# rusty1s/pytorch_sparse

Measured on AMD Instinct MI355X. Metric: SpMM GEdges/s, higher is better.
Workload: dtype f32; 1 GPU; north-star: CSR SpMM 2M x 2M R-MAT ~20 nnz/row, F=128 fp32; reduce=sum, rows_per_gpu=2097152, cols=2097152, edges_per_gpu=40294089, features=128, parallelism=row-sharded x1

## Files before the change

### include/tsamd.h

```cpp
#ifndef TSAMD_H_
#define TSAMD_H_

#include <stddef.h>
#include <stdint.h>

#ifdef __cplusplus
extern "C" {
#endif

typedef enum {
  TSAMD_OK = 0,
  TSAMD_ERR_INVALID = 1,
  TSAMD_ERR_UNSUPPORTED = 2,
  TSAMD_ERR_HIP = 3,
  TSAMD_ERR_WORKSPACE = 4
} tsamd_status;

typedef enum {
  TSAMD_F32 = 0,
  TSAMD_F64 = 1,
  TSAMD_F16 = 2,
  TSAMD_BF16 = 3,
  TSAMD_I32 = 4,
  TSAMD_I64 = 5,
// ... 7 lines not shown
int64_t tsamd_hip_version(void);
int tsamd_build_flags(void);
int tsamd_last_hip_error(void);
const char *tsamd_status_string(int status);

size_t tsamd_spmm_workspace_bytes(int dtype, int reduce, int64_t B, int64_t M,
                                  int64_t N, int64_t K, int64_t E);

int tsamd_spmm_hot_rows_layout(int dtype, int reduce, int64_t B, int64_t M, int64_t N, int64_t K, int64_t E,
                               const void *mat, const void *out, void *workspace, int64_t *layout);

int tsamd_spmm_hot_blocks_layout(int dtype, int reduce, int64_t B, int64_t M, int64_t N, int64_t K, int64_t E,
                                 const void *mat, const void *out, void *workspace, int64_t *layout);
int tsamd_spmm_hot_block_min(void);

int tsamd_spmm_route(int dtype, int reduce, int64_t B, int64_t M, int64_t N, int64_t K, int64_t E, const void *mat,
                     const void *out, const void *arg_out, int arg32, void *workspace, int64_t route[24]);

int tsamd_spmm(int dtype, int reduce, const int64_t *rowptr, const int64_t *col,
               const void *value, const void *mat, void *out, int64_t *arg_out,
               int64_t B, int64_t M, int64_t N, int64_t K, int64_t E,
               void *workspace, size_t workspace_bytes, void *stream);
int tsamd_spmm_reference_order(int set);

int tsamd_spmm_permuted(int dtype, int reduce, const int64_t *rowptr, const int64_t *col,
                        const void *value, const int64_t *perm, const void *mat, void *out,
                        int64_t *arg_out, int64_t B, int64_t M, int64_t N, int64_t K, int64_t E,
                        void *workspace, size_t workspace_bytes, void *stream);

size_t tsamd_spmm_partial_workspace_bytes(int dtype, int reduce, int64_t B, int64_t M, int64_t N, int64_t K,
                                          int64_t E);
int tsamd_spmm_partial(int dtype, int reduce, const int64_t *rowptr, const int64_t *col, const void *value,
                       const void *mat, void *out, int64_t *arg_out, int64_t B, int64_t M, int64_t N, int64_t K,
                       int64_t E, const int64_t *arg_map, int64_t arg_none, int accumulate,
                       const int64_t *deg_rowptr, void *workspace, size_t workspace_bytes, void *stream);

size_t tsamd_spmm_operand_cache_bytes(int dtype, int reduce, int64_t B, int64_t M, int64_t N, int64_t K,
                                      int64_t E);
size_t tsamd_spmm_cached_workspace_bytes(int dtype, int reduce, int64_t B, int64_t M, int64_t N, int64_t K,
                                         int64_t E);
int tsamd_spmm_cached(int dtype, int reduce, const int64_t *rowptr, const int64_t *col, const void *value,
                      const void *mat, void *out, int64_t *arg_out, int64_t B, int64_t M, int64_t N,
                      int64_t K, int64_t E, void *workspace, size_t workspace_bytes, void *cache,
                      size_t cache_bytes, int cache_valid, void *stream);

int tsamd_spmm_profiled(int dtype, int reduce, const int64_t *rowptr,
// ... 349 lines not shown
```

### pytorch_sparse_amd/_native.py

```python
import ctypes
import os

import torch

_HERE = os.path.dirname(os.path.abspath(__file__))
LIB_PATH = os.environ.get('TSAMD_LIB') or os.path.join(_HERE, 'lib', 'libtsamd.so')

SYMBOLS = [
    'tsamd_hip_version', 'tsamd_build_flags', 'tsamd_last_hip_error', 'tsamd_status_string',
    'tsamd_spmm_workspace_bytes', 'tsamd_spmm_hot_rows_layout', 'tsamd_spmm_hot_blocks_layout', 'tsamd_spmm_hot_block_min', 'tsamd_spmm_route', 'tsamd_spmm', 'tsamd_spmm_reference_order', 'tsamd_spmm_permuted', 'tsamd_spmm_profiled',
    'tsamd_spmm_partial_workspace_bytes', 'tsamd_spmm_partial',
    'tsamd_spmm_operand_cache_bytes', 'tsamd_spmm_cached_workspace_bytes', 'tsamd_spmm_cached',
    'tsamd_spmm_minmax_arg32', 'tsamd_spmm_minmax_bw_csc_arg32',
    'tsamd_spmm_minmax_records_in_forward', 'tsamd_spmm_minmax_records_bytes', 'tsamd_spmm_minmax_records_workspace_bytes', 'tsamd_spmm_minmax_records',
    'tsamd_spmm_minmax_winrec', 'tsamd_spmm_minmax_bw_csc_records_workspace_bytes', 'tsamd_spmm_minmax_bw_csc_records',
    'tsamd_gather_rows', 'tsamd_relabel_ids', 'tsamd_spmm_relabelled_workspace_bytes', 'tsamd_spmm_relabelled',
    'tsamd_spmm_coo_small_supported', 'tsamd_spmm_coo_small',
    'tsamd_spmm_value_bw',
    'tsamd_spmm_minmax_bw_workspace_bytes', 'tsamd_spmm_minmax_bw',
    'tsamd_spmm_minmax_bw_csc_workspace_bytes', 'tsamd_spmm_minmax_bw_csc', 'tsamd_spmm_minmax_bw_route',
    'tsamd_ind2ptr', 'tsamd_ptr2ind',
    'tsamd_coo_order', 'tsamd_coo_check', 'tsamd_sort_rank_mode', 'tsamd_sort_route', 'tsamd_sort_coalesce_workspace_bytes', 'tsamd_sort_coalesce', 'tsamd_sort_coalesce_reduce', 'tsamd_sort_coo_workspace_bytes', 'tsamd_sort_coo', 'tsamd_sort_coo_auto', 'tsamd_sort_coo_probed', 'tsamd_sort_coo_values',
    'tsamd_coalesce_workspace_bytes', 'tsamd_coalesce_index', 'tsamd_segment_reduce',
    'tsamd_segment_reduce_balanced_workspace_bytes', 'tsamd_segment_reduce_balanced',
    'tsamd_segment_softmax_route', 'tsamd_segment_softmax_workspace_bytes', 'tsamd_segment_softmax', 'tsamd_segment_softmax_bw',
    'tsamd_sddmm_heads_route', 'tsamd_sddmm_heads', 'tsamd_spmm_heads_route', 'tsamd_spmm_heads_workspace_bytes', 'tsamd_spmm_heads',
    'tsamd_exclusive_scan_workspace_bytes', 'tsamd_exclusive_scan_i64',
    'tsamd_spspmm_route', 'tsamd_spspmm_plan', 'tsamd_spspmm_workspace_bytes', 'tsamd_spspmm_symbolic', 'tsamd_spspmm_numeric',
    'tsamd_spspmm_bw_route', 'tsamd_spspmm_bw_plan_workspace_bytes', 'tsamd_spspmm_bw_workspace_bytes', 'tsamd_spspmm_bw_plan', 'tsamd_spspmm_value_bw',
    'tsamd_index_route', 'tsamd_select_workspace_bytes', 'tsamd_select_plan', 'tsamd_select_fill',
    'tsamd_filter_workspace_bytes', 'tsamd_filter_plan', 'tsamd_filter_apply',
    'tsamd_filter_tiles_workspace_bytes', 'tsamd_filter_count', 'tsamd_filter_write',
    'tsamd_scatter_rows',
# ... 142 lines not shown
    check(st, 'tsamd_spmm')
    return out, arg


SPMM_ROUTE_FIELDS = ('family', 'vec', 'slots', 'lpr', 'lgG', 'ktiles', 'P', 'items', 'snap', 'relabel', 'copy', 'fixup',
                     'table_off', 'tail_row_off', 'head_row_off', 'relabel_flag_off', 'records', 'grid_y',
                     'workspace_bytes')
SPMM_FAMILIES = ('none', 'short', 'cooperative', 'hot_rows', 'hot_blocks', 'arg32_short', 'arg32_cooperative',
                 'reference_order')


def spmm_route(dtype, reduce, B, M, N, K, E, mat=0, out=0, arg_out=0, arg32=False, workspace=0):
    def addr(p):
        return ctypes.c_void_p(int(p.data_ptr() if hasattr(p, 'data_ptr') else p))
    words = (ctypes.c_int64 * 24)()
    st = lib().tsamd_spmm_route(dtype_code(dtype), REDUCES[reduce], _i64(B), _i64(M), _i64(N), _i64(K), _i64(E), addr(mat),
                                addr(out), addr(arg_out), ctypes.c_int(1 if arg32 else 0), addr(workspace), words)
    check(st, 'tsamd_spmm_route')
    r = dict(zip(SPMM_ROUTE_FIELDS, (int(x) for x in words)))
    r['family'] = SPMM_FAMILIES[r['family']]
    return r


def spmm_partial(rowptr, col, value, mat, reduce, out, arg_out=None, arg_map=None, arg_none=0, accumulate=True,
                 deg_rowptr=None):
    require_gpu(rowptr, col, value, mat, out, arg_out, arg_map, deg_rowptr)
    red = REDUCES[reduce]
    dt = dtype_code(mat.dtype)
    if value is not None and value.dtype != mat.dtype:
        raise TsamdError('expected scalar type %s but found %s' % (mat.dtype, value.dtype))
    if not (mat.is_contiguous() and out.is_contiguous() and (arg_out is None or arg_out.is_contiguous())):
        raise TsamdError('tsamd_spmm_partial works in place: mat / out / arg_out must be contiguous')
    if out.dtype != mat.dtype or (red >= 2 and (arg_out is None or arg_out.dtype != torch.int64)):
        raise TsamdError('Input mismatch: out / arg_out')
    M, E = rowptr.numel() - 1, col.numel()
    N, K = mat.size(-2), mat.size(-1)
    B = mat.numel() // max(N * K, 1) if N * K > 0 else 1
    if out.numel() != B * M * K or (arg_out is not None and arg_out.numel() != out.numel()):
        raise TsamdError('Input mismatch: out must be [B, M, K]')
    L = lib()
    nb = L.tsamd_spmm_partial_workspace_bytes(dt, red, _i64(B), _i64(M), _i64(N), _i64(K), _i64(E))
    ws = workspace(nb, mat.device)
    with torch.cuda.device(mat.device):
        st = L.tsamd_spmm_partial(dt, red, _ptr(rowptr), _ptr(col), _ptr(value), _ptr(mat), _ptr(out), _ptr(arg_out),
                                  _i64(B), _i64(M), _i64(N), _i64(K), _i64(E), _ptr(arg_map), _i64(arg_none),
                                  ctypes.c_int(1 if accumulate else 0), _ptr(deg_rowptr), _ptr(ws),
# ... 264 lines not shown
```

### pytorch_sparse_amd/csrc/ops_spmm.cpp

```cpp
#include "ops_common.h"

namespace tsamd_ops {
namespace {

bool stream_is_capturing(void *stream) {
  hipStreamCaptureStatus cs = hipStreamCaptureStatusNone;
  return hipStreamIsCapturing(reinterpret_cast<hipStream_t>(stream), &cs) != hipSuccess ||
         cs != hipStreamCaptureStatusNone;
}

struct TensorIdentity {
  c10::weak_intrusive_ptr<c10::StorageImpl> storage{c10::weak_intrusive_ptr<c10::StorageImpl>(
      c10::make_intrusive<c10::StorageImpl>(c10::StorageImpl::use_byte_size_t(), 0, c10::DataPtr(), nullptr, false))};
  const void *ptr = nullptr;
  uint32_t version = 0;

  static uint32_t version_of(const Tensor &t) { return t.unsafeGetTensorImpl()->version_counter().current_version(); }
  bool matches(const Tensor &t) const {
    if (ptr != t.data_ptr() || version != version_of(t)) return false;
    auto alive = storage.lock();
    return alive && alive.get() == t.storage().unsafeGetStorageImpl();
  }
  void rearm(const Tensor &t) {
    storage = c10::weak_intrusive_ptr<c10::StorageImpl>(
// ... 696 lines not shown

Tensor spmm_coo_small(Tensor index, Tensor value, int64_t M, int64_t N, Tensor mat) {
  if (!(index.device().is_cuda() && value.device().is_cuda() && mat.device().is_cuda()) || mat.dim() != 2 ||
      index.dim() != 2 || index.size(0) != 2 || index.scalar_type() != at::kLong || value.dim() != 1 ||
      value.size(0) != index.size(1) || value.scalar_type() != mat.scalar_type() || mat.size(0) != N ||
      !spmm_coo_small_supported(value, index.size(1), M, mat.size(1)))
    return torch::empty({0}, mat.options().requires_grad(false));
  c10::hip::HIPGuard guard(mat.get_device());
  index = index.contiguous();
  value = value.contiguous();
  mat = mat.contiguous();
  const int64_t E = index.size(1), K = mat.size(1);
  Tensor out = torch::empty({M, K}, mat.options().requires_grad(false));
  check_status(tsamd_spmm_coo_small(dtype_code(mat), index.data_ptr<int64_t>(), index.data_ptr<int64_t>() + E,
                                    value.data_ptr(), mat.data_ptr(), out.data_ptr(), E, M, N, K, current_stream(mat)),
               "tsamd_spmm_coo_small");
  return out;
}

int64_t cuda_version() { return tsamd_hip_version(); }

int64_t reference_order(int64_t set) { return (int64_t)tsamd_spmm_reference_order((int)set); }

bool deterministic_mode() { return at::globalContext().deterministicAlgorithms(); }


}
}

using namespace tsamd_ops;

static auto registry_spmm = torch::RegisterOperators()
                           .op("torch_sparse::spmm_sum", &spmm_sum)
                           .op("torch_sparse::spmm_mean", &spmm_mean)
                           .op("torch_sparse::spmm_min", &spmm_min)
                           .op("torch_sparse::spmm_max", &spmm_max)
                           .op("torch_sparse::ind2ptr", &ind2ptr)
                           .op("torch_sparse::ptr2ind", &ptr2ind)
                           .op("torch_sparse::cuda_version", &cuda_version)
                           .op("tsamd::spmm_coo_small", &spmm_coo_small)
                           .op("tsamd::spmm_coo_small_supported", &spmm_coo_small_supported)
                           .op("tsamd::spmm_minmax", &spmm_minmax)
                           .op("tsamd::deterministic", &deterministic_mode)
                           .op("tsamd::reference_order", &reference_order)
                           .op("tsamd::spmm_sum_owned", &spmm_sum_owned)
                           .op("tsamd::spmm_mean_owned", &spmm_mean_owned)
                           .op("tsamd::operand_cache", &operand_cache_ctl)
                           .op("tsamd::pattern_cache", &pattern_cache_ctl)
                           .op("tsamd::pattern_cache_stats", &pattern_cache_stats)
                           .op("tsamd::relabel_ids", &relabel_ids)
                           .op("tsamd::gather_rows", &gather_rows)
                           .op("tsamd::spmm_relabelled", &spmm_relabelled);
```

### pytorch_sparse_amd/csrc/spmm.hip

```cpp
#define TSAMD_SPMM_PARTIAL_BUILD 0
#include "spmm_kernels.h"

using namespace tsamd;

static int spmm_run(const SpmmCall &c) {
  return spmm_entry(c, [&](int vec, const Workspace &ws) -> int {
    if (c.reduce == TSAMD_MIN) return spmm_launch_min(vec, c, ws);
    if (c.reduce == TSAMD_MAX) return spmm_launch_max(vec, c, ws);
    return TSAMD_DISPATCH_DTYPE_ALL(c.dtype, [&]() -> int { return dispatch_spmm<scalar_t, RED_ADD>(vec, c, ws); });
  });
}

extern "C" size_t tsamd_spmm_workspace_bytes(int dtype, int reduce, int64_t B, int64_t M,
                                             int64_t N, int64_t K, int64_t E) {
  if (dtype_size(dtype) == 0 || B < 0 || M < 0 || N < 0 || K < 0 || E < 0) return 0;
  return carve(nullptr, dtype, reduce, B, M, N, K, E, nullptr);
}

extern "C" int tsamd_spmm(int dtype, int reduce, const int64_t *rowptr, const int64_t *col,
                          const void *value, const void *mat, void *out, int64_t *arg_out,
                          int64_t B, int64_t M, int64_t N, int64_t K, int64_t E, void *workspace,
                          size_t workspace_bytes_given, void *stream_) {
  return spmm_run(SpmmCall{dtype, reduce, rowptr, col, value, mat, out, arg_out, B, M, N, K, E, workspace,
                           workspace_bytes_given, reinterpret_cast<hipStream_t>(stream_)});
// ... 12 lines not shown
  if ((K * es) % packet != 0 || (uintptr_t)mat % packet != 0 || (uintptr_t)out % packet != 0) return 0;
  void *side = nullptr;
  int32_t side_row = 0;
  if (!hot_rows_place(ws, mat, blocks ? N + 64 : N, (uint64_t)K * es, &side, &side_row)) return 0;
  const char *base = reinterpret_cast<const char *>(workspace);
  layout[0] = reinterpret_cast<const char *>(ws.hot_flag) - base;
  layout[1] = reinterpret_cast<const char *>(blocks ? ws.blk_word : ws.hot_word) - base;
  layout[2] = reinterpret_cast<const char *>(side) - base;
  layout[3] = side_row;
  return 1;
}

extern "C" int tsamd_spmm_hot_rows_layout(int dtype, int reduce, int64_t B, int64_t M, int64_t N, int64_t K, int64_t E,
                                          const void *mat, const void *out, void *workspace, int64_t *layout) {
  return hot_layout(false, dtype, reduce, B, M, N, K, E, mat, out, workspace, layout);
}

extern "C" int tsamd_spmm_hot_blocks_layout(int dtype, int reduce, int64_t B, int64_t M, int64_t N, int64_t K, int64_t E,
                                            const void *mat, const void *out, void *workspace, int64_t *layout) {
  return hot_layout(true, dtype, reduce, B, M, N, K, E, mat, out, workspace, layout);
}

extern "C" int tsamd_spmm_hot_block_min(void) { return kHotBlockMin; }

static bool spmm_emits_records(int dtype, int64_t B, int64_t M, int64_t K, int64_t E, const void *mat, const void *out);

int tsamd::spmm_route_words(int dtype, int reduce, int64_t B, int64_t M, int64_t N, int64_t K, int64_t E, const void *mat,
                            const void *out, const void *arg_out, int arg32, void *workspace, bool masked,
                            int64_t route[24]) {
  if (!route || B < 0 || M < 0 || N < 0 || K < 0 || E < 0) return TSAMD_ERR_INVALID;
  for (int i = 0; i < 24; ++i) route[i] = 0;
  if (reduce < TSAMD_SUM || reduce > TSAMD_MAX) return TSAMD_ERR_UNSUPPORTED;
  if (dtype_size(dtype) == 0) return TSAMD_ERR_UNSUPPORTED;
  if (N >= (int64_t)1 << 32 || K >= (int64_t)1 << 31 || B >= 65536) return TSAMD_ERR_UNSUPPORTED;
  if (B * ceil_div(K, 64) >= 65536) return TSAMD_ERR_UNSUPPORTED;
  const bool minmax = reduce == TSAMD_MIN || reduce == TSAMD_MAX;
  const bool floating = dtype == TSAMD_F32 || dtype == TSAMD_F64 || dtype == TSAMD_F16 || dtype == TSAMD_BF16;
  if (arg32 && !minmax) return TSAMD_ERR_UNSUPPORTED;
  if (B * M * K == 0) return TSAMD_OK;
  if (spmm_reference_order_on() && !masked) {
    route[0] = 7;
    return TSAMD_OK;
  }
  if ((uintptr_t)workspace % 256 != 0) return TSAMD_ERR_WORKSPACE;
  if (arg32 && (E >= (int64_t)1 << 31 || !floating)) return TSAMD_ERR_UNSUPPORTED;
  char *base = reinterpret_cast<char *>(workspace);
  if (!base) base = reinterpret_cast<char *>(align_up((size_t)(uintptr_t)mat + 1, 4096));
  if (!mat) mat = base;
  Workspace ws;
  route[18] = (int64_t)carve(base, dtype, reduce, B, M, N, K, E, &ws);
  const int vec = packet_width(dtype, minmax, arg32 != 0, K, mat, out, arg_out);
  const LaneLayout lay = lane_layout(K, vec);
  const size_t es = dtype_size(dtype);
  const int max_vec = es <= 2 ? 4 : (int)(16 / es);
  int mode = ws.xperm != nullptr && vec > 1 ? 2 : 0;
  if (mode == 2 && masked) mode = 1;
  int copy = mode != 0 ? 1 : 0;
  if (mode == 2 && floating && !minmax && vec == max_vec && lay.lgG < 3) {
    void *side = nullptr;
    int32_t side_row = 0;
    if (hot_rows_place(ws, mat, ws.blk_word != nullptr ? N + 64 : N, (uint64_t)K * es, &side, &side_row))
      copy = ws.blk_word != nullptr ? 3 : 2;
  }
  int family;
  if (arg32) family = lay.lgG >= 3 ? 5 : 6;
  else if (lay.lgG >= 3) family = 1;
  else family = copy == 2 ? 3 : (copy == 3 ? 4 : 2);
  route[0] = family;
  route[1] = vec;
  route[2] = lay.slots;
  route[3] = lay.lpr;
  route[4] = lay.lgG;
  route[5] = lay.ktiles;
// ... 214 lines not shown
                                     void *out_h, int64_t *arg_out_h, int64_t B, int64_t M, int64_t N,
                                     int64_t K, int64_t E, void *workspace,
                                     size_t workspace_bytes_given, void *stream_) {
  SpmmCall c{dtype, reduce, rowptr, col_h, value, mat_h, out_h, arg_out_h, B, M, N, K, E, workspace,
             workspace_bytes_given, reinterpret_cast<hipStream_t>(stream_)};
  c.relabelled = true;
  return spmm_run(c);
}

extern "C" int tsamd_spmm_permuted(int dtype, int reduce, const int64_t *rowptr, const int64_t *col,
                                   const void *value, const int64_t *perm, const void *mat, void *out,
                                   int64_t *arg_out, int64_t B, int64_t M, int64_t N, int64_t K,
                                   int64_t E, void *workspace, size_t workspace_bytes_given,
                                   void *stream_) {
  if (E > 0 && !perm) return TSAMD_ERR_INVALID;
  SpmmCall c{dtype, reduce, rowptr, col, value, mat, out, arg_out, B, M, N, K, E, workspace,
             workspace_bytes_given, reinterpret_cast<hipStream_t>(stream_)};
  c.perm = perm;
  return spmm_run(c);
}

namespace tsamd {
size_t spmm_masked_sum_workspace_bytes(int dtype, int64_t B, int64_t M, int64_t N, int64_t K, int64_t E) {
  return carve(nullptr, dtype, TSAMD_SUM, B, M, N, K, E, nullptr);
}
int spmm_masked_sum(int dtype, const int64_t *rowptr, bool has_value, const int64_t *perm,
                    const uint32_t *records, const void *mat, void *out, int64_t B, int64_t M, int64_t N,
                    int64_t K, int64_t E, void *workspace, size_t workspace_bytes, hipStream_t stream) {
  if (E > 0 && !records) return TSAMD_ERR_INVALID;
  const int64_t *col = reinterpret_cast<const int64_t *>(records);
  const void *value = has_value ? reinterpret_cast<const void *>(records) : nullptr;
  SpmmCall c{dtype, TSAMD_SUM, rowptr, col, value, mat, out, nullptr, B, M, N, K, E, workspace,
             workspace_bytes, stream};
  c.perm = perm;
  c.wmask = records;
  return spmm_run(c);
}
}

extern "C" int tsamd_spmm_profiled(int dtype, int reduce, const int64_t *rowptr,
                                   const int64_t *col, const void *value, const void *mat,
                                   void *out, int64_t *arg_out, int64_t B, int64_t M, int64_t N,
                                   int64_t K, int64_t E, void *workspace,
                                   size_t workspace_bytes_given, void *stream_,
                                   float *kernel_ms_host) {
  hipStream_t stream = reinterpret_cast<hipStream_t>(stream_);
  if (!kernel_ms_host) return TSAMD_ERR_INVALID;
// ... 16 lines not shown
```

### pytorch_sparse_amd/csrc/spmm_internal.h

```cpp
#pragma once

#include <hip/hip_runtime.h>
#include <stddef.h>
#include <stdint.h>

namespace tsamd {

struct SpmmCall;
struct Workspace;
int spmm_launch_min(int vec, const SpmmCall &c, const Workspace &ws);
int spmm_launch_max(int vec, const SpmmCall &c, const Workspace &ws);

static inline uint32_t win_record_stride(int64_t K) {
  const uint32_t w = (uint32_t)((K + 31) / 32) + 3u;
  return (w + 3u) & ~3u;
}

static inline int win_record_masked_has_z(uint32_t W) { return (W <= 32u && ((W + 3u) & 3u) != 0u) ? 1 : 0; }

int spmm_route_words(int dtype, int reduce, int64_t B, int64_t M, int64_t N, int64_t K, int64_t E, const void *mat,
                     const void *out, const void *arg_out, int arg32, void *workspace, bool masked, int64_t route[24]);

size_t spmm_masked_sum_workspace_bytes(int dtype, int64_t B, int64_t M, int64_t N, int64_t K, int64_t E);
int spmm_masked_sum(int dtype, const int64_t *rowptr, bool has_value, const int64_t *perm,
                    const uint32_t *records, const void *mat, void *out, int64_t B, int64_t M, int64_t N,
                    int64_t K, int64_t E, void *workspace, size_t workspace_bytes, hipStream_t stream);

int minmax_winrec_from_ids(int dtype, const int64_t *row, const void *value, const int32_t *arg32, uint32_t *records,
                           int64_t B, int64_t M, int64_t K, int64_t E, hipStream_t stream);

bool spmm_reference_order_on();
int spmm_reference_order_run(int dtype, int reduce, const int64_t *rowptr, const int64_t *col, const void *value,
                             const void *mat, void *out, void *arg_out, bool arg32, int64_t B, int64_t M, int64_t N,
                             int64_t K, int64_t E, hipStream_t stream);

}
```

### pytorch_sparse_amd/csrc/spmm_kernels.h

```cpp
#pragma once
#ifndef TSAMD_SPMM_PARTIAL_BUILD
#error "define TSAMD_SPMM_PARTIAL_BUILD as 0 or 1 before including spmm_kernels.h"
#endif

#include "common.h"
#include "scan.h"
#include "spmm_internal.h"

#include <algorithm>
#include <cstdlib>
#include <type_traits>

namespace tsamd {

struct Coord {
  int64_t row;
  int64_t edge;
};

struct Workspace {
  Coord *table;
  int64_t *tail_row;
  int64_t *head_row;
  void *head_val;
// ... 14 lines not shown
  int rec_has_z;
  const unsigned long long *fp_stored, *fp_new;
  unsigned long long *cache_fp;
  int cache_state;
  int partial, accumulate;
  const int64_t *arg_map;
  int64_t arg_none;
  const int64_t *deg_rowptr;
  int arg32;
  uint32_t *rec_out;
  const void *rec_value;
  int64_t snap;
  uint8_t *hot_flag;
  uint32_t *hot_word;
  int64_t *hot_count;
  void *hot_scan;
  void *hot_side;
  int32_t hot_side_row;
  int64_t hot_stride;
  uint32_t *blk_word;
  uint32_t *blk_list;
  uint32_t *blk_total;
  uint32_t blk_chunk;
};

struct SpmmCall {
  int dtype, reduce;
  const int64_t *rowptr, *col;
  const void *value, *mat;
  void *out;
  int64_t *arg_out;
  int64_t B, M, N, K, E;
  void *workspace;
  size_t workspace_bytes;
  hipStream_t stream;
  hipEvent_t *ev = nullptr;
  bool relabelled = false;
  const int64_t *perm = nullptr;
  const uint32_t *wmask = nullptr;
  void *cache = nullptr;
  size_t cache_bytes = 0;
  int cache_valid = 0;
  bool partial = false;
  int accumulate = 0;
  const int64_t *arg_map = nullptr;
  int64_t arg_none = 0;
// ... 295 lines not shown
    if (threadIdx.x == 0) ws.blk_word[w] = r + 1u;
    const uint32_t rot = hot_block_rot(r);
    const int64_t id0 = (int64_t)w * 64;
    const uint64_t from = (uint64_t)id0 << lgS, to = ((uint64_t)r * 64u) << lgS;
    for (uint32_t p0 = threadIdx.x; p0 < packets; p0 += kInFlight * 256) {
      u32x4 v[kInFlight];
      bool on[kInFlight];
#pragma unroll
      for (int t = 0; t < kInFlight; ++t) {
        const uint32_t p = p0 + t * 256;
        on[t] = id0 + (int64_t)(p >> lgS) < N;
        if (on[t]) v[t] = __builtin_nontemporal_load(src + from + p);
      }
#pragma unroll
      for (int t = 0; t < kInFlight; ++t) {
        const uint32_t p = p0 + t * 256;
        const uint32_t row = ((p >> lgS) + rot) & 63u;
        if (on[t]) dst[to + ((uint64_t)row << lgS) + (p & (slots - 1u))] = v[t];
      }
    }
  }
}

__global__ void spmm_partition_kernel(const int64_t *__restrict__ rowptr, int64_t M, int64_t E,
                                      Workspace ws) {
  const int64_t p = (int64_t)blockIdx.x * blockDim.x + threadIdx.x;
  if (p > ws.P) return;
  int64_t d = p * ws.items;
  if (d > M + E) d = M + E;
  int64_t lo = d > E ? d - E : 0;
  int64_t hi = d < M ? d : M;
  while (lo < hi) {
    const int64_t mid = (lo + hi) >> 1;
    if (rowptr[mid + 1] <= d - mid - 1) lo = mid + 1;
    else hi = mid;
  }
  int64_t e = d - lo;
  if (ws.snap > 0 && lo < M) {
    const int64_t rs = rowptr[lo];
    if (e > rs && e - rs <= ws.snap) e = rs;
  }
  ws.table[p] = Coord{lo, e};
}

constexpr uint32_t kNoArg32 = 0xFFFFFFFFu;

template <typename T, int VEC, int RED, typename ARG>
__device__ __forceinline__ void init_acc(typename Traits<T>::acc_t (&val)[VEC], ARG (&arg)[VEC]) {
#pragma unroll
  for (int j = 0; j < VEC; ++j) {
    if constexpr (RED == RED_ADD) val[j] = 0;
    else if constexpr (RED == RED_MIN) val[j] = Traits<T>::max_init();
    else val[j] = Traits<T>::lowest_init();
    arg[j] = (ARG)(sizeof(ARG) == 4 ? (int64_t)kNoArg32 : kNoArg);
  }
}

template <typename T, int VEC>
__device__ __forceinline__ void unpack_packet(const Pack<T, VEC> &x, typename Traits<T>::acc_t (&out)[VEC]) {
  if constexpr (std::is_same<T, bf16_t>::value && VEC % 2 == 0) {
#pragma unroll
    for (int d = 0; d < VEC / 2; ++d) {
      uint32_t word;
      __builtin_memcpy(&word, reinterpret_cast<const char *>(&x) + 4 * d, 4);
      asm volatile("" : "+v"(word));
// ... 387 lines not shown
#endif
constexpr int64_t kFixupRecordMax = TSAMD_FIXUP_RECORD_MAX;

#ifndef TSAMD_RECORD_WAVES
#define TSAMD_RECORD_WAVES 7
#endif
template <int RED, bool SHORT, bool MASKED, int REC = 0>
constexpr int kMinWavesPerEU = kPartial ? ((RED == RED_ADD && !SHORT && !MASKED) ? 8 : 0)
                                        : ((RED != RED_ADD && !SHORT && !MASKED) ? (REC == 1 ? TSAMD_RECORD_WAVES : (REC == 2 ? TSAMD_RECORD_WAVES - 1 : TSAMD_MINMAX_WAVES)) : 0);

template <typename T, int VEC, int RED, bool SHORT, bool MASKED = false, bool A32 = false, int REC = 0, int HOT = 0>
__global__ __launch_bounds__(kWavesPerBlock *kWave, (kMinWavesPerEU<RED, SHORT, MASKED, REC>)) void spmm_merge_kernel(
    const int64_t *__restrict__ rowptr, const int64_t *__restrict__ col,
    const T *__restrict__ value, const T *__restrict__ mat, T *__restrict__ out,
    int64_t *__restrict__ arg_out, int64_t M, int64_t N, uint32_t K, int64_t E,
    uint32_t ktiles, int lgG, bool mean, Workspace ws) {
  using A = typename Traits<T>::acc_t;
  constexpr bool kEmitRecords = REC != 0 && A32 && RED != RED_ADD && !MASKED && !SHORT && VEC == 4 && sizeof(A) == 4 && !kPartial;
  constexpr bool kRec32 = REC == 1;
  static_assert(REC == 0 || kEmitRecords, "record-writing merge kernel: int32 ids, min / max, four-element packets, 4-byte accumulators");
  __shared__ alignas(16) uint32_t rec_tile_[REC == 1 ? kWavesPerBlock * kWave * 4 : (REC == 2 ? kWavesPerBlock * kRecTileWords : 4)];
  const int lane = (int)(threadIdx.x & 63);
  const int wib = __builtin_amdgcn_readfirstlane((int)(threadIdx.x >> 6));
  const int64_t p = (int64_t)blockIdx.x * kWavesPerBlock + wib;
  if (p >= ws.P) return;
  const uint32_t y = blockIdx.y;
  const uint32_t b = y / ktiles;
  const uint32_t kt = y - b * ktiles;

  const Coord c0 = ws.table[p];
  const Coord c1 = ws.table[p + 1];
  const int64_t r0 = c0.row, e0 = c0.edge, r1 = c1.row, e1 = c1.edge;

  const int lpr = 64 >> lgG;
  const int g = lane >> (6 - lgG);
  const int kl = lane & (lpr - 1);
  const uint32_t k0 = (kt * 64u + (uint32_t)kl) * VEC;
  const bool kok = k0 < K;
  static_assert(HOT == 0 || (RED == RED_ADD && !SHORT && !MASKED && !A32 && REC == 0 && !kPartial), "hot rows: plain sums only");
  const bool flagged = use_relabel(ws.relabel_mode, ws.relabel_flag);
  const bool relabel = HOT ? false : flagged;
  const bool hot = HOT ? flagged : false;
  const T *src = relabel ? reinterpret_cast<const T *>(ws.xperm) : mat;
  const T *matk = src + (uint64_t)b * N * K + (kok ? k0 : 0u);
  const uint64_t out_b = (uint64_t)b * M * K + k0;
  const bool writer = g == 0 && kok;
  const uint64_t carry_off = ((uint64_t)b * ws.P + (uint64_t)p) * K + k0;
  const uint32_t *maskk = nullptr;
// ... 677 lines not shown

void plan_partition(int64_t M, int64_t E, int64_t row_bytes, int64_t *P, int64_t *items) {
  const int64_t total = M + E > 0 ? M + E : 1;
  int64_t cap = row_bytes <= 512 ? 256 : (row_bytes < 1024 ? 512 : 1024);
  if (row_bytes <= 128) cap = kShortRowItems;
  if (cap > TSAMD_ITEMS_MAX) cap = TSAMD_ITEMS_MAX;
  int64_t it = ceil_div(total, (int64_t)TSAMD_TARGET_WAVES);
  if (it < TSAMD_ITEMS_MIN) it = TSAMD_ITEMS_MIN;
  if (it > cap) it = cap;
  *items = it;
  *P = ceil_div(total, it);
}


bool relabel_possible(int dtype, int reduce, int64_t N, int64_t K, int64_t E) {
  const int64_t row_bytes = K * (int64_t)dtype_size(dtype);
  const bool size_ok = E >= (1 << 20) && N >= 4096 && N < ((int64_t)1 << 32) && E >= 8 * N &&
                       row_bytes % 16 == 0;
  const bool minmax = reduce == TSAMD_MIN || reduce == TSAMD_MAX;
  const bool camps = row_bytes >= 256 && (row_bytes & (row_bytes - 1)) == 0 && !(minmax && dtype_size(dtype) < 4);
  return size_ok && camps;
}

size_t carve(void *base, int dtype, int reduce, int64_t B, int64_t M, int64_t N, int64_t K,
             int64_t E, Workspace *ws, bool relabelled = false) {
  int64_t P, items;
  plan_partition(M, E, K * (int64_t)dtype_size(dtype), &P, &items);
  const bool minmax = reduce == TSAMD_MIN || reduce == TSAMD_MAX;
  char *p = reinterpret_cast<char *>(base);
  size_t off = 0;
  auto take = [&](size_t bytes) -> void * {
    void *r = p ? p + off : nullptr;
    off += align_up(bytes, 256);
    return r;
  };
  const size_t plane = (size_t)B * P * K;
  Workspace w;
  w.P = P;
  w.items = items;
  w.table = reinterpret_cast<Coord *>(take(sizeof(Coord) * (P + 1)));
  w.tail_row = reinterpret_cast<int64_t *>(take(sizeof(int64_t) * P));
  w.head_val = take(acc_size(dtype) * plane);
  w.tail_val = take(acc_size(dtype) * plane);
  w.head_arg = reinterpret_cast<uint32_t *>(minmax ? take(sizeof(uint32_t) * plane) : nullptr);
  w.tail_arg = reinterpret_cast<uint32_t *>(minmax ? take(sizeof(uint32_t) * plane) : nullptr);
  w.relabel_mode = 0;
  w.relabel_flag = reinterpret_cast<int *>(take(256));
  const bool hot_scope = !relabelled && relabel_possible(dtype, reduce, N, K, E) && !minmax && B == 1 && N < ((int64_t)1 << 31);
  const bool blk_scope = hot_scope && N >= kHotBlockMinN;
  w.xperm = (!relabelled && relabel_possible(dtype, reduce, N, K, E))
                ? take(dtype_size(dtype) * (size_t)B * N * K + (hot_scope ? dtype_size(dtype) * (size_t)K * (blk_scope ? 65 : 1) : 0))
                : nullptr;
  w.head_row = reinterpret_cast<int64_t *>(take(sizeof(int64_t) * P));
  const int64_t hot_words = ceil_div(N, (int64_t)64);
  w.hot_flag = hot_scope ? reinterpret_cast<uint8_t *>(take((size_t)N)) : nullptr;
  w.hot_word = hot_scope ? reinterpret_cast<uint32_t *>(take(16 * (size_t)hot_words)) : nullptr;
  w.hot_count = hot_scope ? reinterpret_cast<int64_t *>(take(sizeof(int64_t) * (size_t)hot_words)) : nullptr;
  w.hot_scan = hot_scope ? take(scan_workspace_bytes(hot_words)) : nullptr;
  w.hot_side = nullptr;
  w.hot_side_row = 0;
  w.hot_stride = TSAMD_HOT_STRIDE;
  w.blk_word = blk_scope ? w.hot_word : nullptr;
  w.blk_list = blk_scope ? w.hot_word + hot_words : nullptr;
  w.blk_total = blk_scope ? reinterpret_cast<uint32_t *>(w.hot_count) : nullptr;
  w.blk_chunk = (uint32_t)(ceil_div(ceil_div(hot_words, (int64_t)kHotChunks), (int64_t)256) * 256);
  w.hash_bits = 1;
  while (w.hash_bits < 32 && ((uint64_t)1 << w.hash_bits) < (uint64_t)(N > 1 ? N : 2)) ++w.hash_bits;
  w.hash_mul = 0x9E3779B1u;
  w.hash_shift = w.hash_bits > 1 ? w.hash_bits / 2 : 1;
  w.out_relabel = 0;
  w.perm = nullptr;
  w.wmask = nullptr;
  w.rec_stride = w.rec_meta = 0;
  w.rec_has_z = 0;
  w.fp_stored = w.fp_new = nullptr;
  w.cache_fp = nullptr;
  w.cache_state = 0;
  w.partial = w.accumulate = 0;
  w.arg_map = nullptr;
  w.arg_none = 0;
  w.deg_rowptr = nullptr;
// ... 6 lines not shown
  w.ohash_shift = w.ohash_bits > 1 ? w.ohash_bits / 2 : 1;
  if (ws) *ws = w;
  return off;
}

constexpr size_t kOperandCacheHeader = 256 + 2 * 512;
size_t operand_cache_bytes(int dtype, int reduce, int64_t B, int64_t N, int64_t K, int64_t E) {
  if (!relabel_possible(dtype, reduce, N, K, E)) return 0;
  return kOperandCacheHeader + align_up(dtype_size(dtype) * (size_t)B * N * K, 256);
}

bool hot_rows_place(const Workspace &ws, const void *mat, int64_t N, uint64_t row_bytes, void **side, int32_t *side_row) {
  if (ws.hot_flag == nullptr || ws.xperm == nullptr || ((uintptr_t)mat % 16) != 0) return false;
  char *xp = reinterpret_cast<char *>(ws.xperm);
  char *at = xp + (((uintptr_t)mat - (uintptr_t)xp) & (row_bytes - 1));
  const int64_t rows = ((int64_t)(intptr_t)at - (int64_t)(intptr_t)mat) / (int64_t)row_bytes;
  const int64_t lim = ((int64_t)1 << 31) - N - 1;
  if (rows > lim || rows < -lim) return false;
  *side = at;
  *side_row = (int32_t)rows;
  return true;
}

template <typename T>
constexpr int kMaxVec = sizeof(T) <= 2 ? 4 : 16 / (int)sizeof(T);

struct LaneLayout {
  uint32_t slots, lpr;
  int lgG;
  uint32_t ktiles;
};
LaneLayout lane_layout(int64_t K, int vec) {
  LaneLayout l;
  l.slots = (uint32_t)((K + vec - 1) / vec);
  l.lpr = l.slots >= 64 ? 64u : (1u << ilog2_ceil(l.slots));
  l.lgG = 6 - ilog2_ceil(l.lpr);
  l.ktiles = (l.slots + 63) / 64;
  return l;
}

[[maybe_unused]] int packet_width(int dtype, bool minmax, bool arg32, int64_t K, const void *mat, const void *out,
                                  const void *arg_out) {
  const size_t es = dtype_size(dtype);
  int vec = es <= 2 ? 4 : (int)(16 / es);
  while (vec > 1 && !((K % vec) == 0 && ((uintptr_t)mat % (vec * es)) == 0 && ((uintptr_t)out % (vec * es)) == 0 &&
                      (!minmax || ((uintptr_t)arg_out % (vec * (arg32 ? 4 : 8))) == 0)))
// ... 68 lines not shown
    } else if (mode != 0) {
      if (cached) {
        hipLaunchKernelGGL(spmm_fingerprint_kernel, dim3(kFingerprintWords), dim3(256), 0, stream,
                           reinterpret_cast<const uint4 *>(mat), (uint64_t)(B * N * K) * sizeof(T) / 16,
                           ws.cache_fp + kFingerprintWords);
        TSAMD_LAUNCH_CHECK();
        if (ws.cache_state == 2) {
          ws.fp_stored = ws.cache_fp;
          ws.fp_new = ws.cache_fp + kFingerprintWords;
        }
      }
      constexpr int kPV = 16 / (int)sizeof(T);
      const uint32_t pslots = (uint32_t)(K / kPV);
      int lgL = 0;
      while (lgL < 8 && (1u << lgL) < pslots) ++lgL;
      hipLaunchKernelGGL((spmm_permute_rows_kernel<T, kPV>), dim3(TSAMD_PERMUTE_BLOCKS), dim3(256), 0, stream, mat,
                         reinterpret_cast<T *>(ws.xperm), B * N, (uint32_t)N, (uint32_t)K, lgL, ws);
      TSAMD_LAUNCH_CHECK();
      if (cached)
        TSAMD_HIP_TRY(hipMemcpyAsync(ws.cache_fp, ws.cache_fp + kFingerprintWords,
                                     sizeof(unsigned long long) * kFingerprintWords, hipMemcpyDeviceToDevice, stream));
    }
  }
  hipLaunchKernelGGL(spmm_partition_kernel, dim3((unsigned int)ceil_div(ws.P + 1, 256)), dim3(256),
                     0, stream, rowptr, M, E, ws);
  TSAMD_LAUNCH_CHECK();
  if (ev) TSAMD_HIP_TRY(hipEventRecord(ev[1], stream));
  const unsigned int gx = (unsigned int)ceil_div(ws.P, kWavesPerBlock);
  constexpr bool kArg32able = !kPartial && RED != RED_ADD &&
                              (std::is_same<T, float>::value || std::is_same<T, double>::value ||
                               std::is_same<T, f16_t>::value || std::is_same<T, bf16_t>::value);
  constexpr bool kMaskable = RED == RED_ADD && (std::is_same<T, float>::value || std::is_same<T, double>::value ||
                                                std::is_same<T, f16_t>::value || std::is_same<T, bf16_t>::value);
  auto merge = [&](auto kernel) {
    hipLaunchKernelGGL(kernel, dim3(gx, (unsigned int)(B * ktiles), 1), dim3(threads), 0, stream, rowptr, col, value, mat,
                       out, arg_out, M, N, (uint32_t)K, E, ktiles, lgG, mean, ws);
  };
  auto fixup = [&](auto kernel) {
    hipLaunchKernelGGL(kernel, dim3(gx, (unsigned int)B, 1), dim3(threads), 0, stream, rowptr, out, arg_out, M, (uint32_t)K,
                       E, mean, ws);
  };
  if (ws.wmask != nullptr) {
    if constexpr (kMaskable)
      merge(spmm_merge_kernel<T, VEC, RED, false, true>);
    else
      return TSAMD_ERR_UNSUPPORTED;
  } else if (kArg32able && ws.arg32) {
    if constexpr (kArg32able) {
      constexpr bool kRecordable = VEC == 4 && sizeof(typename Traits<T>::acc_t) == 4;
// ... 60 lines not shown
  return launch_spmm<T, 1, RED>(c, ws);
}

template <typename Launch>
int spmm_entry(const SpmmCall &c, Launch launch) {
  const int dtype = c.dtype, reduce = c.reduce;
  const int64_t B = c.B, M = c.M, N = c.N, K = c.K, E = c.E;
  if (B < 0 || M < 0 || N < 0 || K < 0 || E < 0) return TSAMD_ERR_INVALID;
  if (reduce < TSAMD_SUM || reduce > TSAMD_MAX) return TSAMD_ERR_UNSUPPORTED;
  if (dtype_size(dtype) == 0) return TSAMD_ERR_UNSUPPORTED;
  if (N >= (int64_t)1 << 32 || K >= (int64_t)1 << 31 || B >= 65536) return TSAMD_ERR_UNSUPPORTED;
  if (B * ceil_div(K, 64) >= 65536) return TSAMD_ERR_UNSUPPORTED;
  const bool minmax = reduce == TSAMD_MIN || reduce == TSAMD_MAX;
  if (B * M * K == 0) return TSAMD_OK;
  if (!c.rowptr || !c.out || (E > 0 && (!c.col || !c.mat)) || (minmax && !c.arg_out))
    return TSAMD_ERR_INVALID;
  if (spmm_reference_order_on() && !c.relabelled && c.perm == nullptr && c.wmask == nullptr && !c.partial)
    return spmm_reference_order_run(dtype, reduce, c.rowptr, c.col, c.value, c.mat, c.out, c.arg_out, c.arg32, B, M, N, K, E,
                                    c.stream);
  const size_t cache_need = operand_cache_bytes(dtype, reduce, B, N, K, E);
  const bool use_cache = c.cache != nullptr && !c.relabelled && cache_need > 0 && c.cache_bytes >= cache_need &&
                         ((uintptr_t)c.cache % 256) == 0 && ((uintptr_t)c.mat % 16) == 0;
  const bool no_xperm_in_ws = c.relabelled || use_cache || c.partial;
  const size_t need = carve(nullptr, dtype, reduce, B, M, N, K, E, nullptr, no_xperm_in_ws);
  if (!c.workspace || c.workspace_bytes < need) return TSAMD_ERR_WORKSPACE;
  if ((uintptr_t)c.workspace % 256 != 0) return TSAMD_ERR_WORKSPACE;
  Workspace ws;
  carve(c.workspace, dtype, reduce, B, M, N, K, E, &ws, no_xperm_in_ws);
  if (use_cache) {
    char *cb = reinterpret_cast<char *>(c.cache);
    ws.relabel_flag = reinterpret_cast<int *>(cb);
    ws.cache_fp = reinterpret_cast<unsigned long long *>(cb + 256);
    ws.xperm = cb + kOperandCacheHeader;
    ws.cache_state = c.cache_valid ? 2 : 1;
  }
  if (c.relabelled) {
    if (M >= (int64_t)1 << 32) return TSAMD_ERR_UNSUPPORTED;
    ws.out_relabel = 1;
  }
  ws.perm = c.perm;
  if (c.arg32) {
    if (!minmax || c.partial || E >= (int64_t)1 << 31) return TSAMD_ERR_UNSUPPORTED;
    ws.arg32 = 1;
    if (c.rec_out != nullptr) {
      ws.rec_out = c.rec_out;
      ws.rec_value = c.value;
      ws.rec_stride = win_record_stride(K);
      ws.rec_meta = (uint32_t)ceil_div(K, 32);
      ws.rec_has_z = ((ws.rec_meta + 3u) & 3u) != 0u ? 1 : 0;
      ws.snap = snap_items(ws.items);
    }
// ... 23 lines not shown
```

Measured before the change: 15.35 GEdges/s.

## Schedule single-row partitions in column-key order to improve gather locality

Adds a per-call reordering of work partitions. Partitions that sit inside one row get a key from their first and last column indices, are bucketed by a histogram, then ranked so that the merge kernel processes them in column order through an indirection array. The aim is to improve L2/MALL reuse of the gathered dense rows. In exchange it adds a memset, two extra kernels and extra workspace on every call, and only applies to sum/mean with wide rows.

```diff
diff --git a/include/tsamd.h b/include/tsamd.h
--- a/include/tsamd.h
+++ b/include/tsamd.h
@@ -53,6 +53,10 @@
                int64_t B, int64_t M, int64_t N, int64_t K, int64_t E,
                void *workspace, size_t workspace_bytes, void *stream);
 int tsamd_spmm_reference_order(int set);
+
+int tsamd_spmm_column_order(int set);
+int tsamd_spmm_order_layout(int dtype, int reduce, int64_t B, int64_t M, int64_t N, int64_t K, int64_t E,
+                            const void *mat, const void *out, void *workspace, int64_t *layout);
 
 int tsamd_spmm_permuted(int dtype, int reduce, const int64_t *rowptr, const int64_t *col,
                         const void *value, const int64_t *perm, const void *mat, void *out,
diff --git a/pytorch_sparse_amd/_native.py b/pytorch_sparse_amd/_native.py
--- a/pytorch_sparse_amd/_native.py
+++ b/pytorch_sparse_amd/_native.py
@@ -8,7 +8,7 @@
 
 SYMBOLS = [
     'tsamd_hip_version', 'tsamd_build_flags', 'tsamd_last_hip_error', 'tsamd_status_string',
-    'tsamd_spmm_workspace_bytes', 'tsamd_spmm_hot_rows_layout', 'tsamd_spmm_hot_blocks_layout', 'tsamd_spmm_hot_block_min', 'tsamd_spmm_route', 'tsamd_spmm', 'tsamd_spmm_reference_order', 'tsamd_spmm_permuted', 'tsamd_spmm_profiled',
+    'tsamd_spmm_workspace_bytes', 'tsamd_spmm_hot_rows_layout', 'tsamd_spmm_hot_blocks_layout', 'tsamd_spmm_hot_block_min', 'tsamd_spmm_route', 'tsamd_spmm', 'tsamd_spmm_reference_order', 'tsamd_spmm_column_order', 'tsamd_spmm_order_layout', 'tsamd_spmm_permuted', 'tsamd_spmm_profiled',
     'tsamd_spmm_partial_workspace_bytes', 'tsamd_spmm_partial',
     'tsamd_spmm_operand_cache_bytes', 'tsamd_spmm_cached_workspace_bytes', 'tsamd_spmm_cached',
     'tsamd_spmm_minmax_arg32', 'tsamd_spmm_minmax_bw_csc_arg32',
@@ -197,6 +197,22 @@
     return r
 
 
+SPMM_ORDER_FIELDS = ('hdr_off', 'order_off', 'P', 'keys_off', 'shift', 'min_singles', 'bucket_max')
+
+
+def spmm_order_layout(dtype, reduce, B, M, N, K, E, mat, out, workspace):
+    def addr(p):
+        return ctypes.c_void_p(int(p.data_ptr() if hasattr(p, 'data_ptr') else p))
+    words = (ctypes.c_int64 * 8)()
+    mode = lib().tsamd_spmm_order_layout(dtype_code(dtype), REDUCES[reduce], _i64(B), _i64(M), _i64(N), _i64(K), _i64(E),
+                                         addr(mat), addr(out), addr(workspace), words)
+    if mode == 0:
+        return None
+    r = dict(zip(SPMM_ORDER_FIELDS, (int(x) for x in words)))
+    r['mode'] = int(mode)
+    return r
+
+
 def spmm_partial(rowptr, col, value, mat, reduce, out, arg_out=None, arg_map=None, arg_none=0, accumulate=True,
                  deg_rowptr=None):
     require_gpu(rowptr, col, value, mat, out, arg_out, arg_map, deg_rowptr)
diff --git a/pytorch_sparse_amd/csrc/ops_spmm.cpp b/pytorch_sparse_amd/csrc/ops_spmm.cpp
--- a/pytorch_sparse_amd/csrc/ops_spmm.cpp
+++ b/pytorch_sparse_amd/csrc/ops_spmm.cpp
@@ -742,6 +742,8 @@
 
 int64_t reference_order(int64_t set) { return (int64_t)tsamd_spmm_reference_order((int)set); }
 
+int64_t column_order(int64_t set) { return (int64_t)tsamd_spmm_column_order((int)set); }
+
 bool deterministic_mode() { return at::globalContext().deterministicAlgorithms(); }
 
 
@@ -763,6 +765,7 @@
                            .op("tsamd::spmm_minmax", &spmm_minmax)
                            .op("tsamd::deterministic", &deterministic_mode)
                            .op("tsamd::reference_order", &reference_order)
+                           .op("tsamd::column_order", &column_order)
                            .op("tsamd::spmm_sum_owned", &spmm_sum_owned)
                            .op("tsamd::spmm_mean_owned", &spmm_mean_owned)
                            .op("tsamd::operand_cache", &operand_cache_ctl)
diff --git a/pytorch_sparse_amd/csrc/spmm.hip b/pytorch_sparse_amd/csrc/spmm.hip
--- a/pytorch_sparse_amd/csrc/spmm.hip
+++ b/pytorch_sparse_amd/csrc/spmm.hip
@@ -1,5 +1,7 @@
 #define TSAMD_SPMM_PARTIAL_BUILD 0
 #include "spmm_kernels.h"
+
+#include <atomic>
 
 using namespace tsamd;
 
@@ -58,6 +60,39 @@
 }
 
 extern "C" int tsamd_spmm_hot_block_min(void) { return kHotBlockMin; }
+
+namespace tsamd {
+namespace {
+std::atomic<int> g_column_order{1};
+}
+int spmm_column_order_mode() { return g_column_order.load(std::memory_order_relaxed); }
+}
+
+extern "C" int tsamd_spmm_column_order(int set) {
+  if (set >= 0 && set <= 2) tsamd::g_column_order.store(set, std::memory_order_relaxed);
+  return tsamd::g_column_order.load(std::memory_order_relaxed);
+}
+
+extern "C" int tsamd_spmm_order_layout(int dtype, int reduce, int64_t B, int64_t M, int64_t N, int64_t K, int64_t E,
+                                       const void *mat, const void *out, void *workspace, int64_t *layout) {
+  if (!layout || !workspace || dtype_size(dtype) == 0 || B < 0 || M < 0 || N < 0 || K < 0 || E < 0) return 0;
+  if (reduce != TSAMD_SUM && reduce != TSAMD_MEAN) return 0;
+  if (B * M * K == 0 || spmm_reference_order_on() || (uintptr_t)workspace % 256 != 0) return 0;
+  Workspace ws;
+  carve(workspace, dtype, reduce, B, M, N, K, E, &ws);
+  const int mode = order_mode_of(ws, dtype, reduce, N, K, E, lane_layout(K, packet_width(dtype, false, false, K, mat, out, nullptr)).lgG);
+  if (mode == 0) return 0;
+  const char *base = reinterpret_cast<const char *>(workspace);
+  layout[0] = reinterpret_cast<const char *>(ws.order_hdr) - base;
+  layout[1] = reinterpret_cast<const char *>(ws.order) - base;
+  layout[2] = ws.P;
+  layout[3] = reinterpret_cast<const char *>(ws.order_cls) - base;
+  layout[4] = ws.order_shift;
+  layout[5] = kOrderMinSingles;
+  layout[6] = kOrderBucketMax;
+  layout[7] = 0;
+  return mode;
+}
 
 static bool spmm_emits_records(int dtype, int64_t B, int64_t M, int64_t K, int64_t E, const void *mat, const void *out);
 
@@ -84,7 +119,7 @@
   if (!base) base = reinterpret_cast<char *>(align_up((size_t)(uintptr_t)mat + 1, 4096));
   if (!mat) mat = base;
   Workspace ws;
-  route[18] = (int64_t)carve(base, dtype, reduce, B, M, N, K, E, &ws);
+  route[18] = (int64_t)carve(base, dtype, reduce, B, M, N, K, E, &ws, false, masked);
   const int vec = packet_width(dtype, minmax, arg32 != 0, K, mat, out, arg_out);
   const LaneLayout lay = lane_layout(K, vec);
   const size_t es = dtype_size(dtype);
@@ -345,7 +380,7 @@
 
 namespace tsamd {
 size_t spmm_masked_sum_workspace_bytes(int dtype, int64_t B, int64_t M, int64_t N, int64_t K, int64_t E) {
-  return carve(nullptr, dtype, TSAMD_SUM, B, M, N, K, E, nullptr);
+  return carve(nullptr, dtype, TSAMD_SUM, B, M, N, K, E, nullptr, false, true);
 }
 int spmm_masked_sum(int dtype, const int64_t *rowptr, bool has_value, const int64_t *perm,
                     const uint32_t *records, const void *mat, void *out, int64_t B, int64_t M, int64_t N,
diff --git a/pytorch_sparse_amd/csrc/spmm_internal.h b/pytorch_sparse_amd/csrc/spmm_internal.h
--- a/pytorch_sparse_amd/csrc/spmm_internal.h
+++ b/pytorch_sparse_amd/csrc/spmm_internal.h
@@ -34,4 +34,6 @@
                              const void *mat, void *out, void *arg_out, bool arg32, int64_t B, int64_t M, int64_t N,
                              int64_t K, int64_t E, hipStream_t stream);
 
+int spmm_column_order_mode();
+
 }
diff --git a/pytorch_sparse_amd/csrc/spmm_kernels.h b/pytorch_sparse_amd/csrc/spmm_kernels.h
--- a/pytorch_sparse_amd/csrc/spmm_kernels.h
+++ b/pytorch_sparse_amd/csrc/spmm_kernels.h
@@ -60,6 +60,15 @@
   uint32_t *blk_list;
   uint32_t *blk_total;
   uint32_t blk_chunk;
+  uint32_t *order_hdr;
+  uint32_t *order;
+  uint32_t *order_cls;
+  uint32_t *order_hist;
+  uint32_t *order_chunk;
+  uint32_t *order_start;
+  uint64_t *order_tmp;
+  uint32_t order_shift;
+  int order_mode;
 };
 
 struct SpmmCall {
@@ -401,8 +410,22 @@
   }
 }
 
-__global__ void spmm_partition_kernel(const int64_t *__restrict__ rowptr, int64_t M, int64_t E,
-                                      Workspace ws) {
+constexpr uint32_t kOrderPad = 0xFFFFFFFFu;
+constexpr int kOrderBuckets = 4096;
+constexpr int kOrderChunkLg = 10;
+constexpr int kOrderHdrWords = 64;
+#ifndef TSAMD_ORDER_MIN_SINGLES
+#define TSAMD_ORDER_MIN_SINGLES 1024
+#endif
+constexpr uint32_t kOrderMinSingles = TSAMD_ORDER_MIN_SINGLES;
+constexpr uint32_t kOrderBucketMax = 16384;
+__device__ __forceinline__ uint32_t order_bucket(uint32_t key, uint32_t shift) {
+  const uint32_t b = key >> shift;
+  return b < (uint32_t)kOrderBuckets ? b : (uint32_t)kOrderBuckets - 1u;
+}
+
+__global__ void spmm_partition_kernel(const int64_t *__restrict__ rowptr, const int64_t *__restrict__ col, int64_t M,
+                                      int64_t E, Workspace ws) {
   const int64_t p = (int64_t)blockIdx.x * blockDim.x + threadIdx.x;
   if (p > ws.P) return;
   int64_t d = p * ws.items;
@@ -420,6 +443,102 @@
     if (e > rs && e - rs <= ws.snap) e = rs;
   }
   ws.table[p] = Coord{lo, e};
+  if (ws.order == nullptr || p >= ws.P) return;
+  uint32_t key = kOrderPad;
+  if (lo < M && e > rowptr[lo]) {
+    int64_t d1 = d + ws.items;
+    if (d1 > M + E) d1 = M + E;
+    if (rowptr[lo + 1] > d1 - lo - 1) key = (uint32_t)col[e] + (uint32_t)col[e + ws.items - 1];
+  }
+  ws.order_cls[p] = key;
+  const bool single = key != kOrderPad;
+  if (single) atomicAdd(&ws.order_hist[order_bucket(key, ws.order_shift)], 1u);
+  const unsigned long long m = __ballot(single);
+  if (m != 0ull && (threadIdx.x & 63) == (unsigned)__builtin_ctzll(__ballot(true)))
+    atomicAdd(&ws.order_chunk[p >> kOrderChunkLg], (uint32_t)__popcll(m));
+}
+
+__device__ __forceinline__ bool order_engaged(int mode, uint32_t P, uint32_t ns, uint32_t maxb) {
+  if (maxb > kOrderBucketMax) return false;
+  return mode == 2 || (ns >= kOrderMinSingles && (uint64_t)ns * 8u >= (uint64_t)P);
+}
+
+__global__ __launch_bounds__(1024) void spmm_order_scatter_kernel(Workspace ws) {
+  __shared__ uint32_t start[kOrderBuckets];
+  __shared__ uint32_t wsum[16], wmax[16], wcnt[16], wpart[16];
+  const uint32_t t = threadIdx.x, lane = t & 63u, wv = t >> 6;
+  const uint32_t P = (uint32_t)ws.P;
+  static_assert(kOrderBuckets == 4096 && kOrderChunkLg == 10, "four buckets per thread, a partition per thread");
+  const uint4 h = reinterpret_cast<const uint4 *>(ws.order_hist)[t];
+  const uint32_t mine = h.x + h.y + h.z + h.w;
+  uint32_t inc = mine, mx = max(max(h.x, h.y), max(h.z, h.w));
+  for (int off = 1; off < 64; off <<= 1) {
+    const uint32_t u = lane_read_u32(inc, lane >= (uint32_t)off ? (int)lane - off : (int)lane);
+    if (lane >= (uint32_t)off) inc += u;
+    mx = max(mx, lane_read_u32(mx, (int)(lane ^ (uint32_t)off)));
+  }
+  if (lane == 63u) wsum[wv] = inc;
+  if (lane == 0u) wmax[wv] = mx;
+  __syncthreads();
+  uint32_t base = 0, ns = 0, maxb = 0;
+  for (uint32_t i = 0; i < 16u; ++i) {
+    base += i < wv ? wsum[i] : 0u;
+    ns += wsum[i];
+    maxb = max(maxb, wmax[i]);
+  }
+  const bool on = order_engaged(ws.order_mode, P, ns, maxb);
+  if (blockIdx.x == 0 && t == 0) {
+    ws.order_hdr[0] = on ? 1u : 0u;
+    ws.order_hdr[1] = ns;
+    ws.order_hdr[2] = maxb;
+  }
+  if (!on) return;
+  const uint32_t s0 = base + inc - mine;
+  const uint4 st = uint4{s0, s0 + h.x, s0 + h.x + h.y, s0 + h.x + h.y + h.z};
+  reinterpret_cast<uint4 *>(start)[t] = st;
+  if (blockIdx.x == 0) reinterpret_cast<uint4 *>(ws.order_start)[t] = st;
+  uint32_t part = 0;
+  for (uint32_t c = t; c < blockIdx.x; c += 1024u) part += ws.order_chunk[c];
+  for (int off = 32; off > 0; off >>= 1) part += lane_read_u32(part, (int)(lane ^ (uint32_t)off));
+  const uint32_t p = blockIdx.x * 1024u + t;
+  const uint32_t key = p < P ? ws.order_cls[p] : kOrderPad;
+  const bool single = key != kOrderPad;
+  const unsigned long long m = __ballot(single);
+  if (lane == 0u) {
+    wcnt[wv] = (uint32_t)__popcll(m);
+    wpart[wv] = part;
+  }
+  __syncthreads();
+  uint32_t before = (uint32_t)__popcll(m & ((1ull << lane) - 1ull));
+  for (uint32_t i = 0; i < 16u; ++i) before += (i < wv ? wcnt[i] : 0u) + wpart[i];
+  if (p < P) {
+    if (!single) {
+      ws.order[p - before] = p;
+    } else {
+      const uint32_t b = order_bucket(key, ws.order_shift);
+      const uint32_t q = start[b] + atomicAdd(&ws.order_hist[kOrderBuckets + b], 1u);
+      ws.order_tmp[q] = ((uint64_t)key << 32) | p;
+    }
+  }
+}
+
+__global__ __launch_bounds__(256) void spmm_order_rank_kernel(Workspace ws) {
+  if (ws.order_hdr[0] == 0u) return;
+  const uint32_t ns = ws.order_hdr[1];
+  const uint32_t lane = threadIdx.x & 63u;
+  const uint32_t first = (uint32_t)__builtin_amdgcn_readfirstlane((int)(blockIdx.x * 4u + (threadIdx.x >> 6)));
+  for (uint32_t i = first; i < ns; i += gridDim.x * 4u) {
+    const uint64_t rec = ws.order_tmp[i];
+    const uint32_t b = order_bucket((uint32_t)(rec >> 32), ws.order_shift);
+    const uint32_t s0 = ws.order_start[b], s1 = s0 + ws.order_hist[b];
+    uint32_t rank = s0;
+    for (uint32_t base = s0; base < s1; base += 64u) {
+      const uint32_t j = base + lane;
+      const bool less = j < s1 && ws.order_tmp[j] < rec;
+      rank += (uint32_t)__popcll(__ballot(less));
+    }
+    if (lane == 0u) ws.order[(uint32_t)ws.P - ns + rank] = (uint32_t)rec;
+  }
 }
 
 constexpr uint32_t kNoArg32 = 0xFFFFFFFFu;
@@ -853,8 +972,14 @@
   __shared__ alignas(16) uint32_t rec_tile_[REC == 1 ? kWavesPerBlock * kWave * 4 : (REC == 2 ? kWavesPerBlock * kRecTileWords : 4)];
   const int lane = (int)(threadIdx.x & 63);
   const int wib = __builtin_amdgcn_readfirstlane((int)(threadIdx.x >> 6));
-  const int64_t p = (int64_t)blockIdx.x * kWavesPerBlock + wib;
+  int64_t p = (int64_t)blockIdx.x * kWavesPerBlock + wib;
   if (p >= ws.P) return;
+  if constexpr (RED == RED_ADD && !SHORT && !MASKED && !A32 && REC == 0 && !kPartial) {
+    if (ws.order != nullptr) {
+      const uint32_t on = ws.order_hdr[0], q = ws.order[p];
+      if (on != 0u) p = (int64_t)q;
+    }
+  }
   const uint32_t y = blockIdx.y;
   const uint32_t b = y / ktiles;
   const uint32_t kt = y - b * ktiles;
@@ -1578,8 +1703,12 @@
   return size_ok && camps;
 }
 
+size_t order_clear_bytes(int64_t P) {
+  return sizeof(uint32_t) * (size_t)(kOrderHdrWords + 2 * kOrderBuckets + ceil_div(P, (int64_t)1 << kOrderChunkLg));
+}
+
 size_t carve(void *base, int dtype, int reduce, int64_t B, int64_t M, int64_t N, int64_t K,
-             int64_t E, Workspace *ws, bool relabelled = false) {
+             int64_t E, Workspace *ws, bool relabelled = false, bool masked = false) {
   int64_t P, items;
   plan_partition(M, E, K * (int64_t)dtype_size(dtype), &P, &items);
   const bool minmax = reduce == TSAMD_MIN || reduce == TSAMD_MAX;
@@ -1613,6 +1742,18 @@
   w.hot_word = hot_scope ? reinterpret_cast<uint32_t *>(take(16 * (size_t)hot_words)) : nullptr;
   w.hot_count = hot_scope ? reinterpret_cast<int64_t *>(take(sizeof(int64_t) * (size_t)hot_words)) : nullptr;
   w.hot_scan = hot_scope ? take(scan_workspace_bytes(hot_words)) : nullptr;
+  const bool order_scope = !relabelled && !masked && !minmax && K * (int64_t)dtype_size(dtype) >= 256 && N < ((int64_t)1 << 31) &&
+                           P < ((int64_t)1 << 31);
+  w.order_hdr = order_scope ? reinterpret_cast<uint32_t *>(take(order_clear_bytes(P))) : nullptr;
+  w.order_hist = order_scope ? w.order_hdr + kOrderHdrWords : nullptr;
+  w.order_chunk = order_scope ? w.order_hist + 2 * kOrderBuckets : nullptr;
+  w.order_start = order_scope ? reinterpret_cast<uint32_t *>(take(sizeof(uint32_t) * kOrderBuckets)) : nullptr;
+  w.order = order_scope ? reinterpret_cast<uint32_t *>(take(sizeof(uint32_t) * (size_t)P)) : nullptr;
+  w.order_cls = order_scope ? reinterpret_cast<uint32_t *>(take(sizeof(uint32_t) * (size_t)P)) : nullptr;
+  w.order_tmp = order_scope ? reinterpret_cast<uint64_t *>(take(sizeof(uint64_t) * (size_t)P)) : nullptr;
+  w.order_shift = 0;
+  while (w.order_shift < 32 && ((uint64_t)(2 * (N > 0 ? N : 1) - 1) >> w.order_shift) >= (uint64_t)kOrderBuckets) ++w.order_shift;
+  w.order_mode = 0;
   w.hot_side = nullptr;
   w.hot_side_row = 0;
   w.hot_stride = TSAMD_HOT_STRIDE;
@@ -1665,6 +1806,15 @@
   return true;
 }
 
+[[maybe_unused]] int order_mode_of(const Workspace &ws, int dtype, int reduce, int64_t N, int64_t K, int64_t E, int lgG) {
+  if (ws.order == nullptr || lgG >= 3 || ws.wmask != nullptr || ws.perm != nullptr || ws.out_relabel || ws.partial ||
+      ws.cache_state != 0 || ws.arg32 || ws.P < 2)
+    return 0;
+  const int sw = spmm_column_order_mode();
+  if (sw == 2) return 2;
+  return sw == 1 && relabel_possible(dtype, reduce, N, K, E) ? 1 : 0;
+}
+
 template <typename T>
 constexpr int kMaxVec = sizeof(T) <= 2 ? 4 : 16 / (int)sizeof(T);
 
@@ -1779,9 +1929,24 @@
                                      sizeof(unsigned long long) * kFingerprintWords, hipMemcpyDeviceToDevice, stream));
     }
   }
+  const int order_mode = !kPartial && RED == RED_ADD ? order_mode_of(ws, c.dtype, c.reduce, N, K, E, lgG) : 0;
+  if (order_mode == 0) {
+    ws.order = nullptr;
+  } else {
+    ws.order_mode = order_mode;
+    TSAMD_HIP_TRY(hipMemsetAsync(ws.order_hdr, 0, order_clear_bytes(ws.P), stream));
+  }
   hipLaunchKernelGGL(spmm_partition_kernel, dim3((unsigned int)ceil_div(ws.P + 1, 256)), dim3(256),
-                     0, stream, rowptr, M, E, ws);
+                     0, stream, rowptr, col, M, E, ws);
   TSAMD_LAUNCH_CHECK();
+  if (order_mode != 0) {
+    hipLaunchKernelGGL(spmm_order_scatter_kernel, dim3((unsigned int)ceil_div(ws.P, (int64_t)1024)), dim3(1024), 0, stream,
+                       ws);
+    TSAMD_LAUNCH_CHECK();
+    hipLaunchKernelGGL(spmm_order_rank_kernel, dim3((unsigned int)std::min<int64_t>(ceil_div(ws.P, (int64_t)4), 2048)), dim3(256),
+                       0, stream, ws);
+    TSAMD_LAUNCH_CHECK();
+  }
   if (ev) TSAMD_HIP_TRY(hipEventRecord(ev[1], stream));
   const unsigned int gx = (unsigned int)ceil_div(ws.P, kWavesPerBlock);
   constexpr bool kArg32able = !kPartial && RED != RED_ADD &&
@@ -1888,11 +2053,11 @@
   const bool use_cache = c.cache != nullptr && !c.relabelled && cache_need > 0 && c.cache_bytes >= cache_need &&
                          ((uintptr_t)c.cache % 256) == 0 && ((uintptr_t)c.mat % 16) == 0;
   const bool no_xperm_in_ws = c.relabelled || use_cache || c.partial;
-  const size_t need = carve(nullptr, dtype, reduce, B, M, N, K, E, nullptr, no_xperm_in_ws);
+  const size_t need = carve(nullptr, dtype, reduce, B, M, N, K, E, nullptr, no_xperm_in_ws, c.wmask != nullptr);
   if (!c.workspace || c.workspace_bytes < need) return TSAMD_ERR_WORKSPACE;
   if ((uintptr_t)c.workspace % 256 != 0) return TSAMD_ERR_WORKSPACE;
   Workspace ws;
-  carve(c.workspace, dtype, reduce, B, M, N, K, E, &ws, no_xperm_in_ws);
+  carve(c.workspace, dtype, reduce, B, M, N, K, E, &ws, no_xperm_in_ws, c.wmask != nullptr);
   if (use_cache) {
     char *cb = reinterpret_cast<char *>(c.cache);
     ws.relabel_flag = reinterpret_cast<int *>(cb);
```

Measured after the change: 17.81 GEdges/s (median of 6 runs). 1.16x the previous value.
